# Corleone-Huang/DynamicVectorQuantization

Measured on AMD Instinct MI355X. Metric: images encoded/sec (VQ hot path: gate + routing + VQ assign), 256x256 inputs, K=1024, higher is better.
Workload: dtype f32; 1 GPU; BASELINE configs[2]: dqvae-entropy-dual-r05, B=256 per GPU, 32x32x256 latents, K=1024, entropy gate + dual routing + VectorQuantize2 assign as one op (quant_conv not in the path); global_batch=256, assign_mode=filter, spinup_steps=100, streams=3, repeats=1, full=False, parallelism=single GPU: no exchange runs, world=1, distinct_devices=1

## Files before the change

dynamicvectorquantization_amd/csrc/dvq_pass1.h:

```cpp
#pragma once
#include "dvq_filter.h"
#include <type_traits>

#define DVQ_LOAD_Z(p) __builtin_nontemporal_load(p)
#define DVQ_STORE_ZQ(p, v) __builtin_nontemporal_store((v), (p))
#define DVQ_BUF_LOAD(rsrc, voff, soff, AUX) __builtin_bit_cast(float, __builtin_amdgcn_raw_buffer_load_b32((rsrc), (voff), (soff), (AUX)))
#define DVQ_BUF_STORE(v, rsrc, voff, soff) __builtin_amdgcn_raw_buffer_store_b32(__builtin_bit_cast(unsigned, (float)(v)), (rsrc), (voff), (soff), 2)
#define DVQ_BUF_LOAD16(XT, rsrc, voff, soff, AUX) dvq_widen_bits<XT>(__builtin_amdgcn_raw_buffer_load_b16((rsrc), (voff), (soff), (AUX)))
#define DVQ_BUF_STORE16(XT, v, rsrc, voff, soff) __builtin_amdgcn_raw_buffer_store_b16(dvq_narrow_bits<XT>(v), (rsrc), (voff), (soff), 2)
#define DVQ_LOAD_SEL(p) (*(p))

#ifdef DVQ_TUNING
#ifdef __HIP_DEVICE_COMPILE__
#define DVQ_TUNING_PTR __device__
#else
#define DVQ_TUNING_PTR static __device__
#endif
DVQ_TUNING_PTR float *g_dvq_tokdbg __asm__("g_dvq_tokdbg") = nullptr;
DVQ_TUNING_PTR unsigned long long *g_dvq_stamps __asm__("g_dvq_stamps") = nullptr;
#define DVQ_STAMP(i) do { if (SPLIT && g_dvq_stamps != nullptr && threadIdx.x == 0) g_dvq_stamps[(size_t)blockIdx.x * 8 + (i)] = wall_clock64(); } while (0)
static inline int dvq_tuning_set_unit(void *stamps, void *tokdbg)
{
    int rc = (int)hipMemcpyToSymbol(HIP_SYMBOL(g_dvq_stamps), &stamps, sizeof(void *));
    if (rc) return rc;
    return (int)hipMemcpyToSymbol(HIP_SYMBOL(g_dvq_tokdbg), &tokdbg, sizeof(void *));
}
#else
#define DVQ_STAMP(i) do { } while (0)
#endif

#define DVQ_SEED_TABLE_TILES 32
constexpr size_t dvq_pass1_lds_bytes(int D) { return 4 * (size_t)(D / 16) * 1024 + 4 * 4 * 64 * sizeof(float) + 4 * 2048; }

template <int D, int SEL, bool CONV, bool FOLD, bool NT, bool RES, bool FLAT = false, bool SPLIT = false, int XT = 0>
__device__ __forceinline__ void pass1_body(
    const float *__restrict__ z, const char *__restrict__ img, const DvqF16Meta *__restrict__ meta,
    const float *__restrict__ E, const float *__restrict__ mask,
    int HW, int K, long N, float *__restrict__ zq, long long *__restrict__ codes,
    double *__restrict__ partials, int *__restrict__ counters, int *__restrict__ exact_list,
    char *__restrict__ records, int rec_cap, const DvqRouted &rv, const DvqConv &cv,
    f32x4 *__restrict__ split = nullptr, int ksplit = 1)
{
    static_assert(!SPLIT || SEL != 2, "the split form: dense or per-lane select; plain, with the conv prologue, or on the folded codebook");
    static_assert(!(SPLIT && FLAT && SEL != 0), "row-major latents are a dense op");
    static_assert(!CONV || (D == 256 && SEL != 2), "the conv prologue exists for D = 256, dense or per-lane select");
    static_assert(!(CONV && FOLD), "the conv is either computed (CONV) or folded into the code image (FOLD)");
    static_assert(!FLAT || (SEL == 0 && !CONV), "the row-major form is a dense op");
    static_assert(XT == 0 || (SEL == 0 && !CONV && !FOLD && !FLAT && !SPLIT), "16-bit latents: the dense lane-per-token form only");
    constexpr int ZB = XT ? 2 : 4;
    constexpr int NW = 4;
    constexpr int S16 = D / 16;
    constexpr int S32 = S16 / 2;
    constexpr int IMG_BYTES = S16 * 1024;
    constexpr int TILE_STRIDE = IMG_BYTES + 256;
    constexpr int CPW = (S16 + NW - 1) / NW;
    static_assert(CPW * NW == S16 && CPW <= 4, "a wave's chunks of a code tile are contiguous and within the instruction offset");
    constexpr int NBUF = 4;
    constexpr int SEED_TILES = NBUF * NW * 64 / 32;
    static_assert(SEED_TILES == DVQ_SEED_TABLE_TILES, "the launcher's limit is the table's size");
    constexpr int PER_TILE = RES ? CPW : CPW + 1;
    constexpr int FLAT_RSH = D * 2 + 16;
    constexpr int FLAT_TRW = 32 * FLAT_RSH;
    constexpr int FLAT_LPT = D * 2 / 16;
    constexpr int FLAT_TPI = 64 / FLAT_LPT;
    constexpr int FLAT_IPH = 32 / FLAT_TPI;
    static_assert(NBUF * IMG_BYTES + NBUF * NW * 64 * 4 + NW * 2048 == dvq_pass1_lds_bytes(D), "the launch's LDS is this carve");
    static_assert(!FLAT || NW * FLAT_TRW <= dvq_pass1_lds_bytes(D), "the images fit the kernel's LDS");
    extern __shared__ __attribute__((aligned(16))) char lds[];
    float *enraw = (float *)(lds + NBUF * IMG_BYTES);
    DVQ_STAMP(0);

    const int tid = threadIdx.x, lane = tid & 63;
    const int wave = __builtin_amdgcn_readfirstlane(tid >> 6);
    const int c = lane & 31, h = lane >> 5;
    const int ks = SPLIT ? (int)(blockIdx.x % (unsigned)ksplit) : 0;
    const int t_lo = SPLIT ? (int)((long)dvq_num_tiles(K) * ks / ksplit) : 0;
    const int T = SPLIT ? (int)((long)dvq_num_tiles(K) * (ks + 1) / ksplit) - t_lo : dvq_num_tiles(K);
    if constexpr (SPLIT) img += (size_t)t_lo * TILE_STRIDE;
    const float sB = meta->scale_b;
    char *scr = lds + NBUF * IMG_BYTES + NBUF * NW * 64 * 4 + wave * 2048;

    auto issue_piece = [&](int t, int q) {
        const int tt = (t < T) ? t : T - 1;
        const char *src = img + (size_t)tt * TILE_STRIDE;
        if (RES || q < CPW) {
            const char *s0 = src + wave * (CPW * 1024) + lane * 16;
            char *d0 = lds + (t & (NBUF - 1)) * IMG_BYTES + wave * (CPW * 1024);
            switch (q) {
            case 0: glds16_off<0>(s0, d0); break;
            case 1: glds16_off<1024>(s0, d0); break;
            case 2: glds16_off<2048>(s0, d0); break;
            default: glds16_off<3072>(s0, d0); break;
            }
        } else {
            glds4(src + IMG_BYTES + lane * 4, enraw + ((t & (NBUF - 1)) * NW + wave) * 64);
        }
    };
    auto issue = [&](int t) {
#pragma unroll
        for (int q = 0; q < PER_TILE; ++q) issue_piece(t, q);
    };
    auto issue_seeds = [&]() {
        if constexpr (RES) {
#pragma unroll
            for (int k = 0; k < SEED_TILES / 2 / NW; ++k) {
                const int pair = wave * (SEED_TILES / 2 / NW) + k;
                const int t0 = (2 * pair < T) ? 2 * pair : T - 1;
                const unsigned voff = (unsigned)c * 4u + ((t0 + 1 < T) ? (unsigned)h * (unsigned)TILE_STRIDE : 0u);
                glds4(img + (size_t)t0 * TILE_STRIDE + IMG_BYTES + voff, enraw + pair * 64);
            }
        }
    };
    const int tile_id = SPLIT ? (int)(blockIdx.x / (unsigned)ksplit) : xcd_swizzle(blockIdx.x, gridDim.x);
    const int pre = (SEL == 2) ? ((rv.G == 2) ? 2 : 1) : 3;

    const int n_raw = (tile_id * NW + wave) * 32 + c;
    const int n = (n_raw < N) ? n_raw : -1;
    auto token_base = [&](int HW, int h) -> size_t {
        const long nn = (n >= 0) ? n : N - 1;
        if constexpr (FLAT) return (size_t)nn * D + 8 * h;
        const long bimg = nn / HW;
        const int hw = (int)(nn - bimg * HW);
        return ((size_t)bimg * D + 8 * h) * HW + hw;
    };
    auto wave_base = [&](const float *p0, int hw, int hh) -> __amdgpu_buffer_rsrc_t {
        const size_t tb = token_base(hw, hh);
        const size_t tb0 = ((size_t)(unsigned)__builtin_amdgcn_readfirstlane((int)(tb >> 32)) << 32) |
                           (size_t)(unsigned)__builtin_amdgcn_readfirstlane((int)(tb & 0xFFFFFFFFu));
        if constexpr (XT != 0) return __builtin_amdgcn_make_buffer_rsrc((void *)((const char *)p0 + tb0 * ZB), 0, -1, 0x00020000);
        else return __builtin_amdgcn_make_buffer_rsrc((void *)(p0 + tb0), 0, -1, 0x00020000);
    };
    auto lane_off = [&](int hw, int hh) -> unsigned {
        const size_t tb = token_base(hw, hh);
        const size_t tb0 = ((size_t)(unsigned)__builtin_amdgcn_readfirstlane((int)(tb >> 32)) << 32) |
                           (size_t)(unsigned)__builtin_amdgcn_readfirstlane((int)(tb & 0xFFFFFFFFu));
        return (unsigned)(tb - tb0) * (XT ? 2u : 4u);
    };
    float zf[S16][8];
    float sel_mask = 1.0f;
    int sel_g = 0;
    unsigned stg_a = 0, stg_b = 0;
    auto conv_prologue = [&](const float *zp, size_t st) __attribute__((always_inline)) {
        constexpr int QIMG = S16 * 1024;
        constexpr int QTILE = 2 * QIMG + 256;
        float *bias_l = enraw;
        float xr[3][8];
        const float *xp = zp;
        auto issue_w = [&](int k, int q) __attribute__((always_inline)) {
            const int i = 4 * wave + q;
            glds16(cv.wimg + (size_t)(i >> 1) * QTILE + (i & 1) * QIMG + k * 1024 + lane * 16,
                   lds + (k & 3) * IMG_BYTES + i * 1024);
        };
        auto issue_x = [&](int k, int j) __attribute__((always_inline)) {
            asm volatile("global_load_dword %0, %1, off nt" : "=v"(xr[k % 3][j]) : "v"(xp) : "memory");
            xp += (j == 7) ? 9 * st : st;
        };
        auto issue_group = [&](int k) __attribute__((always_inline)) {
#pragma unroll
            for (int q = 0; q < 4; ++q) issue_w(k, q);
#pragma unroll
            for (int j = 0; j < 8; ++j) issue_x(k, j);
        };
        glds4(cv.bias + wave * 64 + lane, bias_l + wave * 64);
        issue_group(0);
        issue_group(1);
        issue_group(2);
        f32x16 acc[8];
#pragma unroll
        for (int t8 = 0; t8 < 8; ++t8)
#pragma unroll
            for (int r = 0; r < 16; ++r) acc[t8][r] = 0.0f;
        int ea = 100;
        float sa = ldexpf(1.0f, 100);
        f16x8 xh, xl;
        auto take_group = [&](int g) __attribute__((always_inline)) {
            if (g <= S16 - 3) asm volatile("s_waitcnt vmcnt(24)" ::: "memory");
            else if (g == S16 - 2) asm volatile("s_waitcnt vmcnt(12)" ::: "memory");
            else asm volatile("s_waitcnt vmcnt(0)" ::: "memory");
            float xv[8];
#pragma unroll
            for (int j = 0; j < 8; ++j) { asm volatile("" : "+v"(xr[g % 3][j])); xv[j] = xr[g % 3][j]; }
            float m = 0.0f;
#pragma unroll
            for (int j = 0; j < 8; ++j) m = vmax_abs(m, xv[j]);
            m = fmaxf(m, __shfl_xor(m, 32));
            const bool grow = (m > 0.0f) && (m < __builtin_inff()) && (m * sa >= 32768.0f);
            if (__builtin_amdgcn_ballot_w64(grow) != 0ull) {
                int e;
                (void)frexpf(grow ? m : 1.0f, &e);
                int en = 14 - e;
                en = en > 100 ? 100 : (en < -100 ? -100 : en);
                en = grow ? en : ea;
                if (g > 0) {
                    const float f = ldexpf(1.0f, en - ea);
#pragma unroll
                    for (int t8 = 0; t8 < 8; ++t8)
#pragma unroll
                        for (int r = 0; r < 16; ++r) acc[t8][r] *= f;
                }
                ea = en;
                sa = ldexpf(1.0f, ea);
            }
            u32x4 ph, pl;
#pragma unroll
            for (int j2 = 0; j2 < 4; ++j2) {
                const float v0 = xv[2 * j2] * sa, v1 = xv[2 * j2 + 1] * sa;
                const f32x2 vv = {v0, v1};
                const f16x2 hh = __builtin_convertvector(vv, f16x2);
                const f32x2 rr = {v0 - (float)hh[0], v1 - (float)hh[1]};
                const f16x2 ll = __builtin_convertvector(rr, f16x2);
                ph[j2] = __builtin_bit_cast(unsigned, hh);
                pl[j2] = __builtin_bit_cast(unsigned, ll);
            }
            xh = __builtin_bit_cast(f16x8, ph);
            xl = __builtin_bit_cast(f16x8, pl);
        };
        take_group(0);
#pragma unroll
        for (int s = 0; s < S16; ++s) {
            __builtin_amdgcn_s_barrier();
            asm volatile("" ::: "memory");
            const f16x8 bh = xh, bl = xl;
            const unsigned wa = (unsigned)(size_t)(const __attribute__((address_space(3))) char *)(lds + (s & 3) * IMG_BYTES) + lane * 16;
            f16x8 wf[3];
#define CV_OFF(Q) ((((Q) & 1) ? ((Q) - 1) : ((Q) + 1)) * 1024)
#define CV_RD(Q) asm volatile("ds_read_b128 %0, %1 offset:%c2" : "=v"(wf[(Q) % 3]) : "v"(wa), "i"(CV_OFF(Q)))
#define CV_WAIT(N, Q) asm volatile("s_waitcnt lgkmcnt(" #N ")" : "+v"(wf[(Q) % 3]) :: "memory")
            CV_RD(0); CV_RD(1); CV_RD(2);
            __builtin_amdgcn_sched_barrier(0);
#define CV_TILE(T8, W0, W1)                                                                                              \
            CV_WAIT(W0, 2 * (T8));                                                                                        \
            __builtin_amdgcn_sched_barrier(0);                                                                            \
            acc[T8] = __builtin_amdgcn_mfma_f32_32x32x16_f16(wf[(2 * (T8)) % 3], bh, acc[T8], 0, 0, 0);    \
            __builtin_amdgcn_sched_barrier(0);                                                                            \
            if (2 * (T8) + 3 < 16) { CV_RD(2 * (T8) + 3 < 16 ? 2 * (T8) + 3 : 0); }                                       \
            CV_WAIT(W1, 2 * (T8) + 1);                                                                                    \
            __builtin_amdgcn_sched_barrier(0);                                                                            \
            acc[T8] = __builtin_amdgcn_mfma_f32_32x32x16_f16(wf[(2 * (T8) + 1) % 3], bl, acc[T8], 0, 0, 0);               \
            acc[T8] = __builtin_amdgcn_mfma_f32_32x32x16_f16(wf[(2 * (T8) + 1) % 3], bh, acc[T8], 0, 0, 0);               \
            __builtin_amdgcn_sched_barrier(0);                                                                            \
            if (2 * (T8) + 4 < 16) { CV_RD(2 * (T8) + 4 < 16 ? 2 * (T8) + 4 : 0); }
#define CV_W(Q) if (s + 3 < S16) { issue_w(s + 3, Q); __builtin_amdgcn_sched_barrier(0); }
#define CV_X(J) if (s + 3 < S16) { issue_x(s + 3, J); issue_x(s + 3, (J) + 1); __builtin_amdgcn_sched_barrier(0); }
            CV_TILE(0, 2, 2) CV_W(0) CV_TILE(1, 2, 2) CV_W(1) CV_TILE(2, 2, 2) CV_W(2) CV_TILE(3, 2, 2) CV_W(3)
            CV_TILE(4, 2, 2) CV_X(0) CV_TILE(5, 2, 2) CV_X(2) CV_TILE(6, 2, 2) CV_X(4) CV_TILE(7, 1, 0) CV_X(6)
#undef CV_W
#undef CV_X
#undef CV_TILE
#undef CV_WAIT
#undef CV_RD
#undef CV_OFF
            __builtin_amdgcn_sched_barrier(0);
            if (s + 1 < S16) take_group(s + 1);
        }
        const float unscale = ldexpf(cv.meta->inv_scale_w, -ea);
#pragma unroll
        for (int s = 0; s < S16; ++s) {
            const f32x4 b0 = *(const f32x4 *)(bias_l + 16 * s + 8 * h), b1v = *(const f32x4 *)(bias_l + 16 * s + 8 * h + 4);
#pragma unroll
            for (int j = 0; j < 8; ++j)
                zf[s][j] = __builtin_fmaf(acc[s >> 1][8 * (s & 1) + j], unscale, (j < 4) ? b0[j & 3] : b1v[j & 3]);
            __builtin_amdgcn_sched_barrier(0);
        }
        if (cv.h_all && n >= 0) {
            float *hp = cv.h_buf + token_base(HW, h);
#pragma unroll
            for (int s = 0; s < S16; ++s)
#pragma unroll
                for (int j = 0; j < 8; ++j) hp[(size_t)(16 * s + j) * HW] = zf[s][j];
        }
        __builtin_amdgcn_s_barrier();
        asm volatile("" ::: "memory");
        issue_seeds();
        for (int t = 0; t < 3; ++t) issue(t);
        __builtin_amdgcn_sched_barrier(0);
    };
    if (SEL != 0) {
        const int nn = (n >= 0) ? n : (int)(N - 1);
        const int b = nn / HW, pos = nn - b * HW;
        const int y = pos / rv.Wout, x = pos - y * rv.Wout;
        const int SC = rv.sub[rv.G - 1];
        const size_t cell = (size_t)b * rv.hc * rv.wc + (y / SC) * rv.wc + x / SC;
        const DvqGateRaw graw = dvq_gate_fetch(rv.gate, rv.gate_mode, rv.G, cell);
        auto by_products = [&](int g) {
            const int rep_g = rv.rep[g];
            sel_mask = 1.0f / (float)(rep_g * rep_g);
            if (n >= 0 && h == 0 && rv.cmask_out != nullptr) {
                rv.cmask_out[n] = sel_mask;
                if (y % SC == 0 && x % SC == 0) {
                    rv.indices_out[cell] = g;
                    if (rv.gate_mode == 2 && rv.gate_out != nullptr) {
                        const float e = graw.f[0];
                        longlong2 gg; gg.x = (e <= rv.thr) ? 1 : 0; gg.y = (e > rv.thr) ? 1 : 0;
                        *(longlong2 *)(rv.gate_out + 2 * cell) = gg;
                    }
                }
            }
            if (!(y % rep_g == 0 && x % rep_g == 0)) sel_mask = -sel_mask;
        };
        if (SEL == 1) {
            const int g = dvq_gate_reduce(graw, rv.gate_mode, rv.G, rv.thr);
            by_products(g);
            int stride_l;
            const float *zp = dvq_dense_source(rv, b, y, x, g, stride_l) + (size_t)8 * h * stride_l;
            const size_t st = (size_t)stride_l;
            if constexpr (CONV) {
                conv_prologue(zp, st);
            } else {
            issue_seeds();
            for (int t = 0; t < pre; ++t) issue(t);
            __builtin_amdgcn_s_setprio(2);
#pragma unroll
            for (int s = 0; s < S16; ++s)
#pragma unroll
                for (int j = 0; j < 8; ++j) zf[s][j] = DVQ_LOAD_SEL(zp + (size_t)(16 * s + j) * st);
            __builtin_amdgcn_s_setprio(0);
            }
        } else {
            issue_seeds();
            for (int t = 0; t < pre; ++t) issue(t);
            const int bw = __builtin_amdgcn_readfirstlane(b);
            const int y0 = __builtin_amdgcn_readfirstlane(y) - wave;
            char *img_a = lds + pre * IMG_BYTES;
            char *img_b = lds + 3 * IMG_BYTES;
            {
                const int ga = rv.G - 2;
                const int plane = rv.hc * rv.sub[ga] * 16;
                const float *src = rv.src[ga] + (size_t)bw * D * plane + (size_t)(y0 >> 1) * 16 + (lane & 7) * 4;
                for (int i = wave; i < D / 8; i += NW)
                    glds16(src + (size_t)(i * 8 + (lane >> 3)) * plane, img_a + i * 1024);
            }
            if (rv.G == 3) {
                const int plane = rv.hc * 8;
                const float *src = rv.src[0] + (size_t)bw * D * plane + (size_t)(y0 >> 2) * 8 + (lane & 1) * 4;
                for (int i = wave; i < D / 32; i += NW)
                    glds16(src + (size_t)(i * 32 + (lane >> 1)) * plane, img_b + i * 1024);
            }
            stg_a = (unsigned)(size_t)(const __attribute__((address_space(3))) char *)img_a +
                    (unsigned)((8 * h) * 128 + (((wave >> 1) * 16 + (c >> 1)) << 2));
            stg_b = (unsigned)(size_t)(const __attribute__((address_space(3))) char *)img_b +
                    (unsigned)((8 * h) * 32 + ((c >> 2) << 2));
            const __amdgpu_buffer_rsrc_t zr = __builtin_amdgcn_make_buffer_rsrc((void *)(rv.src[rv.G - 1] + (size_t)bw * D * HW), 0,
                                                                                -1, 0x00020000);
            const unsigned zo = (unsigned)(8 * h * HW + pos) * 4u;
            __builtin_amdgcn_s_setprio(2);
#pragma unroll
            for (int s = 0; s < S16; ++s)
#pragma unroll
                for (int j = 0; j < 8; ++j) zf[s][j] = DVQ_BUF_LOAD(zr, zo, (16 * s + j) * HW * 4, NT ? 2 : 0);
            __builtin_amdgcn_s_setprio(0);
            asm volatile("s_waitcnt vmcnt(0)" ::: "memory");
            __builtin_amdgcn_s_barrier();
            asm volatile("" ::: "memory");
            sel_g = dvq_gate_reduce(graw, rv.gate_mode, rv.G, rv.thr);
            by_products(sel_g);
        }
    } else if constexpr (CONV) {
        conv_prologue(z + token_base(HW, h), (size_t)HW);
    } else if constexpr (FLAT) {
        char *tr = lds + wave * FLAT_TRW;
        const long n0 = ((long)tile_id * NW + wave) * 32;
        f32x4 tmp[2][FLAT_IPH];
#pragma unroll
        for (int h2 = 0; h2 < 2; ++h2)
#pragma unroll
            for (int i = 0; i < FLAT_IPH; ++i) {
                long tk = n0 + i * FLAT_TPI + lane / FLAT_LPT;
                tk = tk < N ? tk : N - 1;
                const f32x4 *src = (const f32x4 *)(z + (size_t)tk * D + h2 * (D / 2)) + (lane % FLAT_LPT);
                tmp[h2][i] = NT ? __builtin_nontemporal_load(src) : *src;
            }
#pragma unroll
        for (int h2 = 0; h2 < 2; ++h2) {
#pragma unroll
            for (int i = 0; i < FLAT_IPH; ++i)
                *(f32x4 *)(tr + (i * FLAT_TPI + lane / FLAT_LPT) * FLAT_RSH + (lane % FLAT_LPT) * 16) = tmp[h2][i];
#pragma unroll
            for (int sp = 0; sp < S16 / 2; ++sp) {
                const int s = h2 * (S16 / 2) + sp;
                const f32x4 lo = *(const f32x4 *)(tr + c * FLAT_RSH + (16 * sp + 8 * h) * 4);
                const f32x4 hi = *(const f32x4 *)(tr + c * FLAT_RSH + (16 * sp + 8 * h + 4) * 4);
#pragma unroll
                for (int j = 0; j < 4; ++j) { zf[s][j] = lo[j]; zf[s][4 + j] = hi[j]; }
            }
        }
        __syncthreads();
        issue_seeds();
        for (int t = 0; t < pre; ++t) issue(t);
    } else {
        issue_seeds();
        for (int t = 0; t < pre; ++t) issue(t);
        const __amdgpu_buffer_rsrc_t zr = wave_base(z, HW, h);
        const unsigned zo = lane_off(HW, h);
        __builtin_amdgcn_s_setprio(2);
#pragma unroll
        for (int s = 0; s < S16; ++s)
#pragma unroll
            for (int j = 0; j < 8; ++j) {
                if constexpr (XT != 0) zf[s][j] = DVQ_BUF_LOAD16(XT, zr, zo, (16 * s + j) * HW * 2, NT ? 2 : 0);
                else zf[s][j] = DVQ_BUF_LOAD(zr, zo, (16 * s + j) * HW * 4, NT ? 2 : 0);
            }
        __builtin_amdgcn_s_setprio(0);
    }
    f16x8 zb[2][S32];
    float xn, thr2W;
    unsigned copymask = 0u;
    unsigned perm_off[2] = {0u, 0u};
    if constexpr (SEL == 2) {
        copymask = (unsigned)__builtin_amdgcn_ballot_w64(sel_mask < 0.0f && h == 0);
        const int below = __builtin_popcount(copymask & ((1u << c) - 1u));
        const int p = (sel_mask < 0.0f) ? 32 - __builtin_popcount(copymask) + below : c - below;
        unsigned char *tab = (unsigned char *)scr;
        if (h == 0) tab[p] = (unsigned char)c;
#pragma unroll
        for (int t2 = 0; t2 < 2; ++t2) {
            const unsigned col = tab[16 * t2 + (lane & 15)];
            perm_off[t2] = (unsigned)(lane >> 5) * 1024u + (col + 32u * ((unsigned)(lane >> 4) & 1u)) * 16u;
        }
    }
    {
        float pa[2][8];
        float amax = 0.0f, zeta2 = 0.0f;
        f16x8 zprev = {};
#pragma unroll
        for (int s = 0; s < S16; ++s) {
            if (SEL == 2) {
                if (sel_g == rv.G - 2) {
#pragma unroll
                    for (int j = 0; j < 8; ++j)
                        asm volatile("ds_read_b32 %0, %1 offset:%c2" : "+v"(zf[s][j]) : "v"(stg_a), "i"((16 * s + j) * 128));
                    asm volatile("s_waitcnt lgkmcnt(0)" ::: "memory");
                }
                if (rv.G == 3 && sel_g == 0) {
#pragma unroll
                    for (int j = 0; j < 8; ++j)
                        asm volatile("ds_read_b32 %0, %1 offset:%c2" : "+v"(zf[s][j]) : "v"(stg_b), "i"((16 * s + j) * 32));
                    asm volatile("s_waitcnt lgkmcnt(0)" ::: "memory");
                }
#pragma unroll
                for (int j = 0; j < 8; ++j) asm volatile("" : "+v"(zf[s][j]));
            }
            u32x4 packed;
#pragma unroll
            for (int j2 = 0; j2 < 4; ++j2) {
                const float v0 = zf[s][2 * j2], v1 = zf[s][2 * j2 + 1];
                const float q0 = sq_rn(v0), q1 = sq_rn(v1);
                pa[s & 1][2 * j2] = (s < 2) ? q0 : __fadd_rn(pa[s & 1][2 * j2], q0);
                pa[s & 1][2 * j2 + 1] = (s < 2) ? q1 : __fadd_rn(pa[s & 1][2 * j2 + 1], q1);
                amax = vmax_abs(amax, v0);
                amax = vmax_abs(amax, v1);
                f32x2 vv = {v0, v1};
                f16x2 hh = __builtin_convertvector(vv, f16x2);
                packed[j2] = __builtin_bit_cast(unsigned, hh);
                const float r0 = v0 - (float)hh[0], r1 = v1 - (float)hh[1];
                zeta2 = __builtin_fmaf(r0, r0, zeta2);
                zeta2 = __builtin_fmaf(r1, r1, zeta2);
            }
            if constexpr (SEL == 2) {
                asm volatile("" : "+v"(packed), "+v"(zeta2));
                if (sel_mask < 0.0f) packed = u32x4{0u, 0u, 0u, 0u};
            }
            const f16x8 zcur = __builtin_bit_cast(f16x8, packed);
            if (s & 1) {
                const int sp = s >> 1;
                *(f16x8 *)(scr + lane * 16) = zprev;
                *(f16x8 *)(scr + 1024 + lane * 16) = zcur;
#pragma unroll
                for (int t2 = 0; t2 < 2; ++t2) {
                    if constexpr (SEL == 2) {
                        zb[t2][sp] = *(const f16x8 *)(scr + perm_off[t2]);
                    } else {
                    const int srcl = 16 * t2 + (lane & 15) + 32 * ((lane >> 4) & 1);
                    zb[t2][sp] = *(const f16x8 *)(scr + (lane >> 5) * 1024 + srcl * 16);
                    }
                }
            }
            zprev = zcur;
            if constexpr (CONV) __builtin_amdgcn_sched_barrier(0);
        }
        float t8[8];
#pragma unroll
        for (int l = 0; l < 8; ++l) {
            float o0 = __shfl_xor(pa[0][l], 32), o1 = __shfl_xor(pa[1][l], 32);
            float a0 = h == 0 ? pa[0][l] : o0;
            float a1 = h == 0 ? o0 : pa[0][l];
            float a2 = h == 0 ? pa[1][l] : o1;
            float a3 = h == 0 ? o1 : pa[1][l];
            t8[l] = __fadd_rn(__fadd_rn(__fadd_rn(a0, a1), a2), a3);
        }
        xn = t8[0];
#pragma unroll
        for (int l = 1; l < 8; ++l) xn = __fadd_rn(xn, t8[l]);
        amax = fmaxf(amax, __shfl_xor(amax, 32));
        zeta2 += __shfl_xor(zeta2, 32);
        thr2W = FOLD ? dvq_fold_threshold(xn, amax, zeta2, sB, (const DvqFoldMeta *)meta)
                     : dvq_filter_threshold(xn, amax, zeta2, sB, meta);
    }
    if (SEL == 2) {
        __builtin_amdgcn_s_barrier();
        asm volatile("" ::: "memory");
    }
    for (int t = pre; t < 3; ++t) issue(t);
    DVQ_STAMP(1);

    float best, second;
    int code;
    {
        const int q16 = lane >> 4;
        float b1[2] = {-__builtin_inff(), -__builtin_inff()}, b2[2] = {-__builtin_inff(), -__builtin_inff()};
        int bt[2] = {0, 0};
        if constexpr (SEL == 2) {
            if (__builtin_popcount(copymask) >= 16) {
#define DVQ_NG 1
#include "pass1_loop.h"
#undef DVQ_NG
            } else {
#define DVQ_NG 2
#include "pass1_loop.h"
#undef DVQ_NG
            }
        } else {
#define DVQ_NG 2
#include "pass1_loop.h"
#undef DVQ_NG
        }
        asm volatile("s_waitcnt vmcnt(0)" ::: "memory");
        float rb[2], rs[2];
        int rc[2];
#pragma unroll
        for (int t2 = 0; t2 < 2; ++t2) {
            float mb = b1[t2], ms = b2[t2];
            int mt = bt[t2], mq = q16;
#pragma unroll
            for (int off = 16; off <= 32; off <<= 1) {
                const float o1 = __shfl_xor(mb, off), o2 = __shfl_xor(ms, off);
                const int ot = __shfl_xor(mt, off), oq = __shfl_xor(mq, off);
                const bool other_wins = (o1 > mb) || (o1 == mb && ((lane ^ off) < lane));
                ms = fmaxf(other_wins ? mb : o1, fmaxf(ms, o2));
                mb = other_wins ? o1 : mb;
                mt = other_wins ? ot : mt;
                mq = other_wins ? oq : mq;
            }
            const int r = (int)(__float_as_uint(mb) & 15u);
            rb[t2] = mb;
            rs[t2] = ms;
            rc[t2] = (mt + t_lo) * 32 + 16 * (r >> 2) + 4 * mq + (r & 3);
        }
        if constexpr (SEL == 2) {
            unsigned cm = copymask;
            asm volatile("" : "+s"(cm));
            const int c_p = (int)__builtin_amdgcn_mbcnt_hi(~0u, __builtin_amdgcn_mbcnt_lo(~0u, 0u)) & 31;
            const int below = __builtin_popcount(cm & ((1u << c_p) - 1u));
            const int pc = ((cm >> c_p) & 1u) ? 32 - __builtin_popcount(cm) + below : c_p - below;
            const int srcl = pc & 15;
            const float x0 = __shfl(rb[0], srcl), x1 = __shfl(rb[1], srcl);
            const float y0 = __shfl(rs[0], srcl), y1 = __shfl(rs[1], srcl);
            const int c0 = __shfl(rc[0], srcl), c1 = __shfl(rc[1], srcl);
            best = (pc >> 4) ? x1 : x0;
            second = (pc >> 4) ? y1 : y0;
            code = (pc >> 4) ? c1 : c0;
        } else {
        const int srcl = c & 15;
        const float x0 = __shfl(rb[0], srcl), x1 = __shfl(rb[1], srcl);
        const float y0 = __shfl(rs[0], srcl), y1 = __shfl(rs[1], srcl);
        const int c0 = __shfl(rc[0], srcl), c1 = __shfl(rc[1], srcl);
        best = (c >> 4) ? x1 : x0;
        second = (c >> 4) ? y1 : y0;
        code = (c >> 4) ? c1 : c0;
        }
    }
    DVQ_STAMP(2);
    if constexpr (SEL == 2) {
        const int lane_e = (int)__builtin_amdgcn_mbcnt_hi(~0u, __builtin_amdgcn_mbcnt_lo(~0u, 0u));
        const int c_e = lane_e & 31;
        float am = __builtin_fabsf(sel_mask);
        asm volatile("" : "+v"(am));
        const int rm1 = (am == 1.0f) ? 0 : ((am == 0.25f) ? 1 : 3);
        char *hand = lds + NBUF * IMG_BYTES + NBUF * NW * 64 * 4;
        if (lane_e < 32) {
            const f32x4 mine = {best, second, __int_as_float(code), 0.0f};
            *(f32x4 *)(hand + wave * 2048 + c_e * 16) = mine;
        }
        __syncthreads();
        const f32x4 own = *(const f32x4 *)(hand + (wave - (wave & rm1)) * 2048 + (c_e - (c_e & rm1)) * 16);
        best = own[0];
        second = own[1];
        code = __float_as_int(own[2]);
    }
    if constexpr (SPLIT) {
        typedef __attribute__((address_space(1))) unsigned long long gu64;
        __shared__ int s_last;
        gu64 *mine = (gu64 *)(split + ((size_t)tile_id * ksplit) * 128 + wave * 32 + c);
        if (h == 0) {
            gu64 *e = mine + (size_t)ks * 128 * 2;
            __hip_atomic_store(e, ((unsigned long long)__float_as_uint(second) << 32) | __float_as_uint(best), __ATOMIC_RELAXED, __HIP_MEMORY_SCOPE_AGENT);
            __hip_atomic_store(e + 1, (unsigned long long)(unsigned)code, __ATOMIC_RELAXED, __HIP_MEMORY_SCOPE_AGENT);
        }
        asm volatile("s_waitcnt vmcnt(0)" ::: "memory");
        __syncthreads();
        DVQ_STAMP(3);
        if (tid == 0) {
            const int old = __hip_atomic_fetch_add(&counters[DVQ_SPLIT_TICKET0 + tile_id], 1, __ATOMIC_RELAXED, __HIP_MEMORY_SCOPE_AGENT);
            s_last = (old == ksplit - 1);
            if (old == ksplit - 1)
                __hip_atomic_store(&counters[DVQ_SPLIT_TICKET0 + tile_id], 0, __ATOMIC_RELAXED, __HIP_MEMORY_SCOPE_AGENT);
        }
        __syncthreads();
        DVQ_STAMP(4);
        if (!s_last) return;
        float mb = -__builtin_inff(), ms = -__builtin_inff();
        int mc = 0;
        unsigned long long e0[DVQ_SPLIT_MAX_SLICES], e1[DVQ_SPLIT_MAX_SLICES];
#pragma unroll
        for (int k = 0; k < DVQ_SPLIT_MAX_SLICES; ++k) {
            const int kk = k < ksplit ? k : ksplit - 1;
            e0[k] = __hip_atomic_load(mine + (size_t)kk * 128 * 2, __ATOMIC_RELAXED, __HIP_MEMORY_SCOPE_AGENT);
            e1[k] = __hip_atomic_load(mine + (size_t)kk * 128 * 2 + 1, __ATOMIC_RELAXED, __HIP_MEMORY_SCOPE_AGENT);
        }
#pragma unroll
        for (int k = 0; k < DVQ_SPLIT_MAX_SLICES; ++k) {
            const float eb = __uint_as_float((unsigned)e0[k]), es = __uint_as_float((unsigned)(e0[k] >> 32));
            const bool other_wins = k < ksplit && eb > mb;
            ms = (k < ksplit) ? fmaxf(other_wins ? mb : eb, fmaxf(ms, es)) : ms;
            mc = other_wins ? (int)(unsigned)e1[k] : mc;
            mb = other_wins ? eb : mb;
        }
        best = mb; second = ms; code = mc;
        DVQ_STAMP(5);
    }
    const float thr = best - thr2W;
    const bool final_ok = (best - second) > thr2W;
    const bool valid = n >= 0;
    bool hopeless = !(code < K) || !(thr == thr);
#ifdef DVQ_TUNING
    if (g_dvq_tokdbg != nullptr && valid && h == 0) {
        f32x4 dbg = {best, second, thr2W, (float)code};
        *(f32x4 *)(g_dvq_tokdbg + 4 * (size_t)n) = dbg;
    }
#endif
    const bool undecided = valid && !hopeless && !final_ok;
    const int sel_rep = (SEL == 0 || sel_mask < 0.0f) ? (SEL == 0 ? 1 : 0) : (sel_mask == 1.0f ? 1 : (sel_mask == 0.25f ? 2 : 4));
    const bool queued = undecided && sel_rep > 0;
    const unsigned long long umask = __ballot(queued && h == 0);
    const int shard = (SPLIT ? tile_id * NW + wave : (int)blockIdx.x) & (DVQ_QSHARDS - 1);
    int slot_raw = 0;
    if (umask != 0ull && lane == 0) slot_raw = atomicAdd(&counters[DVQ_QCOUNT0 + shard], (int)__popcll(umask));
    if (valid && hopeless && h == 0) {
        int pos = atomicAdd(&counters[DVQ_C_EXACT], 1);
        exact_list[pos] = n;
    }
    float lsum = 0.0f;
    float m_tok = 1.0f;
    if (valid && !hopeless) {
        if (h == 0) codes[n] = (long long)code;
        m_tok = (SEL != 0) ? __builtin_fabsf(sel_mask) : ((mask != nullptr) ? mask[n] : 1.0f);
        if (zq != nullptr || partials != nullptr) {
            int h_e = h;
            if constexpr (FOLD || (FLAT && SPLIT) || SEL == 2) h_e =(int)(__builtin_amdgcn_mbcnt_hi(~0u, __builtin_amdgcn_mbcnt_lo(~0u, 0u)) >> 5);
            const float *ep = E + (size_t)code * D + 8 * h_e;
            constexpr int SB = SPLIT ? ((S16 < 8) ? S16 : 8) : ((S16 < 2) ? S16 : 2);
            auto finish = [&](auto store_tag) {
                constexpr bool STORE = decltype(store_tag)::value;
                int hw_e = HW;
                asm volatile("" : "+s"(hw_e));
                const __amdgpu_buffer_rsrc_t qr = wave_base(STORE ? zq : (float *)E, hw_e, h_e);
                const unsigned qo = lane_off(hw_e, h_e);
                int hw4 = HW * (XT ? 2 : 4);
                asm volatile("" : "+s"(hw4));
#pragma unroll
                for (int s0 = 0; s0 < S16; s0 += SB) {
                    f32x4 eg[SB][2];
#pragma unroll
                    for (int q = 0; q < SB; ++q) {
                        eg[q][0] = *(const f32x4 *)(ep + 16 * (s0 + q));
                        eg[q][1] = *(const f32x4 *)(ep + 16 * (s0 + q) + 4);
                    }
#pragma unroll
                    for (int q = 0; q < SB; ++q) {
                        const int s = s0 + q;
#pragma unroll
                        for (int j = 0; j < 8; ++j) {
                            float e = eg[q][j >> 2][j & 3];
                            if constexpr (FOLD) {
                                if (STORE) DVQ_BUF_STORE(e, qr, qo, (16 * s + j) * hw4);
                            } else {
                            float diff = __fsub_rn(e, zf[s][j]);
                            if constexpr (XT != 0) {
                                if (STORE) DVQ_BUF_STORE16(XT, __fadd_rn(zf[s][j], diff), qr, qo, (16 * s + j) * hw4);
                            } else
                            if (STORE) DVQ_BUF_STORE(__fadd_rn(zf[s][j], diff), qr, qo, (16 * s + j) * hw4);
                            lsum = __builtin_fmaf(diff, diff, lsum);
                            }
                        }
                    }
                }
            };
            if constexpr (!FLAT) {
                if (zq != nullptr) finish(std::true_type{});
                else finish(std::false_type{});
                lsum *= m_tok;
            }
        }
    }
    if constexpr (FLAT) {
        char *flat_tr = lds + wave * FLAT_TRW;
        const bool store = zq != nullptr;
        if (store) __syncthreads();
        const bool mine = valid && !hopeless && (store || partials != nullptr);
        const unsigned long long okmask = __ballot(valid && !hopeless && h == 0);
        const long n0 = ((long)tile_id * NW + wave) * 32;
        const float *ep = E + (size_t)(mine ? code : 0) * D + 8 * h;
#pragma unroll
        for (int h2 = 0; h2 < 2; ++h2) {
            if (mine) {
                constexpr int SB = (S16 / 2 < 2) ? S16 / 2 : 2;
#pragma unroll
                for (int sp0 = 0; sp0 < S16 / 2; sp0 += SB) {
                    f32x4 eg[SB][2];
#pragma unroll
                    for (int q = 0; q < SB; ++q) {
                        eg[q][0] = *(const f32x4 *)(ep + 16 * (h2 * (S16 / 2) + sp0 + q));
                        eg[q][1] = *(const f32x4 *)(ep + 16 * (h2 * (S16 / 2) + sp0 + q) + 4);
                    }
#pragma unroll
                    for (int q = 0; q < SB; ++q) {
                        const int sp = sp0 + q, s = h2 * (S16 / 2) + sp;
                        f32x4 o[2];
#pragma unroll
                        for (int j = 0; j < 8; ++j) {
                            const float e = eg[q][j >> 2][j & 3];
                            if constexpr (FOLD) {
                                o[j >> 2][j & 3] = e;
                            } else {
                                const float diff = __fsub_rn(e, zf[s][j]);
                                o[j >> 2][j & 3] = __fadd_rn(zf[s][j], diff);
                                lsum = __builtin_fmaf(diff, diff, lsum);
                            }
                        }
                        if (store) {
                            *(f32x4 *)(flat_tr + c * FLAT_RSH + (16 * sp + 8 * h) * 4) = o[0];
                            *(f32x4 *)(flat_tr + c * FLAT_RSH + (16 * sp + 8 * h + 4) * 4) = o[1];
                        }
                    }
                }
            }
            if (store) {
#pragma unroll
                for (int i = 0; i < FLAT_IPH; ++i) {
                    const int tk = i * FLAT_TPI + lane / FLAT_LPT;
                    const f32x4 v = *(const f32x4 *)(flat_tr + tk * FLAT_RSH + (lane % FLAT_LPT) * 16);
                    if ((okmask >> tk) & 1ull)
                        __builtin_nontemporal_store(v, (f32x4 *)(zq + (size_t)(n0 + tk) * D + h2 * (D / 2)) + (lane % FLAT_LPT));
                }
            }
        }
        lsum *= m_tok;
    }
    DVQ_STAMP(6);
    if (umask != 0ull) {
        const int base = __shfl(slot_raw, 0);
        int slot = base + (int)__popcll(umask & ((1ull << c) - 1ull));
        slot = queued ? slot : -1;
        if (queued && slot >= rec_cap) {
            if (h == 0) {
                const int rr = sel_rep > 0 ? sel_rep : 1;
                for (int ry = 0; ry < rr; ++ry)
                    for (int rx = 0; rx < rr; ++rx) {
                        int pos = atomicAdd(&counters[DVQ_C_EXACT], 1);
                        exact_list[pos] = n + ry * rv.Wout + rx;
                    }
            }
            lsum = -(float)(sel_rep * sel_rep - 1) * lsum;
            slot = -1;
        }
        if (slot >= 0) {
            char *rec = records + ((size_t)shard * rec_cap + slot) * rec_bytes(D);
#pragma unroll
            for (int s = 0; s < S16; ++s) {
                f32x4 lo = {zf[s][0], zf[s][1], zf[s][2], zf[s][3]};
                f32x4 hi = {zf[s][4], zf[s][5], zf[s][6], zf[s][7]};
                *(f32x4 *)(rec + (16 * s + 8 * h) * 4) = lo;
                *(f32x4 *)(rec + (16 * s + 8 * h + 4) * 4) = hi;
            }
            if (h == 0) {
                RecMeta rm;
                rm.n = n; rm.xn = xn; rm.thr = thr; rm.m = m_tok; rm.prov = code;
                rm.best = ~0ull; rm.rep = sel_rep > 0 ? sel_rep : 1;
                *(RecMeta *)(rec + (size_t)D * 4) = rm;
            }
        }
    }
    if (partials != nullptr) {
        double dsum = (double)lsum;
#pragma unroll
        for (int off = 32; off > 0; off >>= 1) dsum += __shfl_xor(dsum, off);
        __syncthreads();
        double *red = (double *)lds;
        if (lane == 0) red[wave] = dsum;
        __syncthreads();
        if (tid == 0) partials[SPLIT ? tile_id : (int)blockIdx.x] = (red[0] + red[1]) + (red[2] + red[3]);
    }
    DVQ_STAMP(7);
}

template <int D, int SEL, bool CONV, bool FOLD, bool RES>
__global__ __launch_bounds__(256, 2) void vq_assign_filter_kernel(
    const float *__restrict__ z, const char *__restrict__ img, const DvqF16Meta *__restrict__ meta,
    const float *__restrict__ E, const float *__restrict__ mask,
    int HW, int K, long N, float *__restrict__ zq, long long *__restrict__ codes,
    double *__restrict__ partials, int *__restrict__ counters, int *__restrict__ exact_list,
    char *__restrict__ records, int rec_cap, const DvqRouted rv, const DvqConv cv)
{
    pass1_body<D, SEL, CONV, FOLD, true, RES>(z, img, meta, E, mask, HW, K, N, zq, codes, partials, counters, exact_list, records, rec_cap, rv, cv);
}

template <int D, bool FOLD, bool RES>
__global__ __launch_bounds__(256, 2) void vq_assign_filter_flat_kernel(
    const float *__restrict__ z, const char *__restrict__ img, const DvqF16Meta *__restrict__ meta,
    const float *__restrict__ E, const float *__restrict__ mask,
    int HW, int K, long N, float *__restrict__ zq, long long *__restrict__ codes,
    double *__restrict__ partials, int *__restrict__ counters, int *__restrict__ exact_list,
    char *__restrict__ records, int rec_cap, const DvqRouted rv, const DvqConv cv)
{
    pass1_body<D, 0, false, FOLD, true, RES, true>(z, img, meta, E, mask, HW, K, N, zq, codes, partials, counters, exact_list, records, rec_cap, rv, cv);
}

template <int D, int SEL, bool CONV, bool FOLD, bool FLAT, bool RES>
__global__ __launch_bounds__(256, 2) void vq_assign_filter_split_kernel(
    const float *__restrict__ z, const char *__restrict__ img, const DvqF16Meta *__restrict__ meta,
    const float *__restrict__ E, const float *__restrict__ mask,
    int HW, int K, long N, float *__restrict__ zq, long long *__restrict__ codes,
    double *__restrict__ partials, int *__restrict__ counters, int *__restrict__ exact_list,
    char *__restrict__ records, int rec_cap, const DvqRouted rv, const DvqConv cv, f32x4 *__restrict__ split, int ksplit)
{
    pass1_body<D, SEL, CONV, FOLD, CONV, RES, FLAT, true>(z, img, meta, E, mask, HW, K, N, zq, codes, partials, counters, exact_list, records,
                                                     rec_cap, rv, cv, split, ksplit);
}

template <int D, int SEL, bool FOLD, bool RES>
__global__ __launch_bounds__(256, 2) void vq_assign_filter_cached_kernel(
    const float *__restrict__ z, const char *__restrict__ img, const DvqF16Meta *__restrict__ meta,
    const float *__restrict__ E, const float *__restrict__ mask,
    int HW, int K, long N, float *__restrict__ zq, long long *__restrict__ codes,
    double *__restrict__ partials, int *__restrict__ counters, int *__restrict__ exact_list,
    char *__restrict__ records, int rec_cap, const DvqRouted rv, const DvqConv cv)
{
    pass1_body<D, SEL, false, FOLD, false, RES>(z, img, meta, E, mask, HW, K, N, zq, codes, partials, counters, exact_list, records, rec_cap, rv, cv);
}

template <int D, bool RES, int XT>
__global__ __launch_bounds__(256, 2) void vq_assign_filter_x16_kernel(
    const void *__restrict__ z, const char *__restrict__ img, const DvqF16Meta *__restrict__ meta,
    const float *__restrict__ E, const float *__restrict__ mask,
    int HW, int K, long N, void *__restrict__ zq, long long *__restrict__ codes,
    double *__restrict__ partials, int *__restrict__ counters, int *__restrict__ exact_list,
    char *__restrict__ records, int rec_cap)
{
    static_assert(XT == 1 || XT == 2, "f16 or bf16");
    pass1_body<D, 0, false, false, true, RES, false, false, XT>((const float *)z, img, meta, E, mask, HW, K, N, (float *)zq, codes, partials,
                                                                counters, exact_list, records, rec_cap, DvqRouted{}, DvqConv{});
}

struct FilterWs {
    int *counters, *chunk_sync, *exact_list;
    char *records;
    int cap;
    f32x4 *split;
};

enum class P1Form { plain, cached, flat, split, wide, x16 };
struct P1Plan {
    P1Form form;
    int sel;
    bool conv, fold, flat;
    int ks;
    int xt;
};

constexpr bool p1_keeps_seed_piece(int D, P1Form form, bool fold, bool flat)
{
    return D == 256 && ((form == P1Form::flat && fold) || (form == P1Form::split && flat));
}

struct P1Args {
    const float *z;
    const char *img16;
    const DvqF16Meta *meta;
    const float *E, *mask;
    int HW, K;
    long N;
// ... 103 lines not shown
```

dynamicvectorquantization_amd/csrc/pass1_loop.h:

```cpp
        f32x4 acc16[2][2];
        auto top2 = [&](int tt) {
#pragma unroll
            for (int t2 = 0; t2 < DVQ_NG; ++t2) {
                const float om = b1[t2];
#pragma unroll
                for (int r = 0; r < 8; r += 2) {
                    const float v0 = acc16[r >> 2][t2][r & 3], v1 = acc16[(r + 1) >> 2][t2][(r + 1) & 3];
                    float g0 = __uint_as_float((__float_as_uint(v0) & 0xFFFFFFF0u) | (unsigned)r);
                    float g1 = __uint_as_float((__float_as_uint(v1) & 0xFFFFFFF0u) | (unsigned)(r + 1));
                    float md = __builtin_amdgcn_fmed3f(b1[t2], g0, g1);
                    b1[t2] = vmax3_raw(b1[t2], g0, g1);
                    b2[t2] = vmax_raw(b2[t2], md);
                }
                bt[t2] = (b1[t2] != om) ? tt : bt[t2];
            }
        };
    for (int t = 0; t < T; ++t) {
            asm volatile("s_waitcnt vmcnt(%0)" ::"n"(PER_TILE) : "memory");
            __builtin_amdgcn_s_barrier();
            asm volatile("" ::: "memory");
            if (S16 != 16) issue(t + 3);
            const unsigned tile_a = (unsigned)(size_t)(const __attribute__((address_space(3))) char *)(
                                        lds + (t & (NBUF - 1)) * IMG_BYTES + lane * 16);
            f16x8 a0, a1, a2, a3;
#define DVQ_RD(dst, S) asm volatile("ds_read_b128 %0, %1 offset:%c2" : "=v"(dst) : "v"(tile_a), "i"((S) * 1024))
            DVQ_RD(a0, 0); DVQ_RD(a1, 1); DVQ_RD(a2, 2); DVQ_RD(a3, 3);
            __builtin_amdgcn_sched_barrier(0);
            if (t > 0) top2(t - 1);
            __builtin_amdgcn_sched_barrier(0);
            {
                const unsigned seed_a = (unsigned)(size_t)(const __attribute__((address_space(3))) char *)(
                                            RES ? enraw + t * 32 + 4 * q16 : enraw + ((t & (NBUF - 1)) * NW + wave) * 64 + 4 * q16);
                f32x4 e0, e1;
                asm volatile("ds_read_b128 %0, %1" : "=v"(e0) : "v"(seed_a));
                asm volatile("ds_read_b128 %0, %1 offset:64" : "=v"(e1) : "v"(seed_a));
                asm volatile("s_waitcnt lgkmcnt(0)" : "+v"(e0), "+v"(e1), "+v"(a0), "+v"(a1), "+v"(a2), "+v"(a3) :: "memory");
                acc16[0][0] = e0; if (DVQ_NG == 2) acc16[0][1] = e0;
                acc16[1][0] = e1; if (DVQ_NG == 2) acc16[1][1] = e1;
            }
            __builtin_amdgcn_sched_barrier(0);
#define DVQ_PIECE(Q) if constexpr ((Q) < PER_TILE) { issue_piece(t + 3, Q); }
#define DVQ_MM(src, F, WAIT, NEXT)                                                                             \
            asm volatile("s_waitcnt lgkmcnt(" #WAIT ")" ::: "memory");                                            \
            __builtin_amdgcn_sched_barrier(0);                                                                    \
            acc16[(F) / S32][0] = __builtin_amdgcn_mfma_f32_16x16x32_f16(src, zb[0][(F) % S32], acc16[(F) / S32][0], 0, 0, 0); \
            if (DVQ_NG == 2)                                                                                      \
            acc16[(F) / S32][1] = __builtin_amdgcn_mfma_f32_16x16x32_f16(src, zb[1][(F) % S32], acc16[(F) / S32][1], 0, 0, 0); \
            __builtin_amdgcn_sched_barrier(0);                                                                    \
            if ((F) + 4 < S16) { DVQ_RD(src, ((F) + 4 < S16 ? (F) + 4 : 0)); }                                  \
            NEXT
            __builtin_amdgcn_s_setprio(1);
            if (S16 == 16) {
                DVQ_MM(a0, 0, 0, ) DVQ_MM(a1, 1, 1, DVQ_PIECE(0)) DVQ_MM(a2, 2, 2, ) DVQ_MM(a3, 3, 3, )
                DVQ_MM(a0, 4, 3, DVQ_PIECE(1)) DVQ_MM(a1, 5, 3, ) DVQ_MM(a2, 6, 3, ) DVQ_MM(a3, 7, 3, DVQ_PIECE(2))
                DVQ_MM(a0, 8, 3, ) DVQ_MM(a1, 9, 3, ) DVQ_MM(a2, 10, 3, DVQ_PIECE(3)) DVQ_MM(a3, 11, 3, )
                DVQ_MM(a0, 12, 3, ) DVQ_MM(a1, 13, 2, DVQ_PIECE(4)) DVQ_MM(a2, 14, 1, ) DVQ_MM(a3, 15, 0, )
            } else if (S16 == 8) {
                DVQ_MM(a0, 0, 0, ) DVQ_MM(a1, 1, 1, ) DVQ_MM(a2, 2, 2, ) DVQ_MM(a3, 3, 3, )
                DVQ_MM(a0, 4, 3, ) DVQ_MM(a1, 5, 2, ) DVQ_MM(a2, 6, 1, ) DVQ_MM(a3, 7, 0, )
            } else {
                DVQ_MM(a0, 0, 0, ) DVQ_MM(a1, 1, 0, ) DVQ_MM(a2, 2, 0, ) DVQ_MM(a3, 3, 0, )
            }
#undef DVQ_MM
#undef DVQ_RD
#undef DVQ_PIECE
            __builtin_amdgcn_s_setprio(0);
        }
        top2(T - 1);
```

Measured before the change: 1.343 million images/s.

## Compact real tokens across the workgroup to skip MFMA work for copied tokens

For the SEL==2, D==256 path, each wave publishes its copy-token mask to shared memory. Real (non-copied) tokens are then compacted across all four waves through an LDS exchange buffer, so each wave runs the codebook distance loop only on its share of the compacted tokens (0, 1 or 2 MFMA groups). Results are scattered back through LDS to the owning lanes. This removes wasted MFMA work when many tokens are duplicates, at the cost of extra workgroup barriers and LDS traffic in the transpose and hand-back phases.

```diff
diff --git a/dynamicvectorquantization_amd/csrc/dvq_pass1.h b/dynamicvectorquantization_amd/csrc/dvq_pass1.h
--- a/dynamicvectorquantization_amd/csrc/dvq_pass1.h
+++ b/dynamicvectorquantization_amd/csrc/dvq_pass1.h
@@ -112,7 +112,18 @@
         }
     };
     const int tile_id = SPLIT ? (int)(blockIdx.x / (unsigned)ksplit) : xcd_swizzle(blockIdx.x, gridDim.x);
+    constexpr bool WGC = (SEL == 2 && D == 256);
     const int pre = (SEL == 2) ? ((rv.G == 2) ? 2 : 1) : 3;
+    char *const xbuf_a = lds + NBUF * IMG_BYTES + NBUF * NW * 64 * 4;
+    char *xbuf_b = nullptr;
+    if constexpr (WGC) xbuf_b = lds + pre * IMG_BYTES;
+    static_assert(!WGC || (64 * 128 == 8192 && S32 >= 4), "channels 0 .. 63 of the [D][32 floats] image are the second buffer");
+    unsigned wgm0 = 0u, wgm1 = 0u, wgm2 = 0u, wgm3 = 0u;
+    unsigned *wg_masks = nullptr;
+    if constexpr (WGC) {
+        __shared__ unsigned s_wg_masks[4];
+        wg_masks = s_wg_masks;
+    }
 
     const int n_raw = (tile_id * NW + wave) * 32 + c;
     const int n = (n_raw < N) ? n_raw : -1;
@@ -349,11 +360,24 @@
 #pragma unroll
                 for (int j = 0; j < 8; ++j) zf[s][j] = DVQ_BUF_LOAD(zr, zo, (16 * s + j) * HW * 4, NT ? 2 : 0);
             __builtin_amdgcn_s_setprio(0);
+            if constexpr (WGC) {
+                sel_g = dvq_gate_reduce(graw, rv.gate_mode, rv.G, rv.thr);
+                const int rep_g = rv.rep[sel_g];
+                const unsigned cm = (unsigned)__builtin_amdgcn_ballot_w64(!(y % rep_g == 0 && x % rep_g == 0) && h == 0);
+                if (lane == 0) wg_masks[wave] = cm;
+                asm volatile("s_waitcnt vmcnt(0) lgkmcnt(0)" ::: "memory");
+            } else
             asm volatile("s_waitcnt vmcnt(0)" ::: "memory");
             __builtin_amdgcn_s_barrier();
             asm volatile("" ::: "memory");
-            sel_g = dvq_gate_reduce(graw, rv.gate_mode, rv.G, rv.thr);
+            if constexpr (!WGC) sel_g = dvq_gate_reduce(graw, rv.gate_mode, rv.G, rv.thr);
             by_products(sel_g);
+            if constexpr (WGC) {
+                wgm0 = (unsigned)__builtin_amdgcn_readfirstlane((int)wg_masks[0]);
+                wgm1 = (unsigned)__builtin_amdgcn_readfirstlane((int)wg_masks[1]);
+                wgm2 = (unsigned)__builtin_amdgcn_readfirstlane((int)wg_masks[2]);
+                wgm3 = (unsigned)__builtin_amdgcn_readfirstlane((int)wg_masks[3]);
+            }
         }
     } else if constexpr (CONV) {
         conv_prologue(z + token_base(HW, h), (size_t)HW);
@@ -406,6 +430,32 @@
     float xn, thr2W;
     unsigned copymask = 0u;
     unsigned perm_off[2] = {0u, 0u};
+    int ng = 2;
+    if constexpr (WGC) {
+        const int nr0 = 32 - __builtin_popcount(wgm0), nr1 = 32 - __builtin_popcount(wgm1), nr2 = 32 - __builtin_popcount(wgm2);
+        const int pf1 = nr0, pf2 = pf1 + nr1, pf3 = pf2 + nr2, nreal_wg = pf3 + 32 - __builtin_popcount(wgm3);
+        const int left = nreal_wg - 32 * wave + 15;
+        ng = __builtin_amdgcn_readfirstlane(left < 16 ? 0 : (left < 32 ? 1 : 2));
+        const int wz = wgm0 ? 0 : (wgm1 ? 1 : (wgm2 ? 2 : 3));
+        const unsigned mz = wgm0 ? wgm0 : (wgm1 ? wgm1 : (wgm2 ? wgm2 : wgm3));
+        const int cz = mz ? __builtin_ctz(mz) : 0;
+#pragma unroll
+        for (int t2 = 0; t2 < 2; ++t2) {
+            const int P = 32 * wave + 16 * t2 + (lane & 15);
+            const int ws = (P >= pf3) ? 3 : ((P >= pf2) ? 2 : ((P >= pf1) ? 1 : 0));
+            int k = P - ((P >= pf3) ? pf3 : ((P >= pf2) ? pf2 : ((P >= pf1) ? pf1 : 0)));
+            const unsigned real = ~((ws == 3) ? wgm3 : ((ws == 2) ? wgm2 : ((ws == 1) ? wgm1 : wgm0)));
+            int col = 0;
+#pragma unroll
+            for (int sh = 16; sh >= 1; sh >>= 1) {
+                const int cnt = __builtin_popcount((real >> col) & ((1u << sh) - 1u));
+                if (k >= cnt) { k -= cnt; col += sh; }
+            }
+            const bool past = P >= nreal_wg;
+            const unsigned wsrc = past ? (unsigned)wz : (unsigned)ws, csrc = past ? (unsigned)cz : (unsigned)col;
+            perm_off[t2] = wsrc * 2048u + (unsigned)(lane >> 5) * 1024u + (csrc + 32u * ((unsigned)(lane >> 4) & 1u)) * 16u;
+        }
+    } else
     if constexpr (SEL == 2) {
         copymask = (unsigned)__builtin_amdgcn_ballot_w64(sel_mask < 0.0f && h == 0);
         const int below = __builtin_popcount(copymask & ((1u << c) - 1u));
@@ -463,6 +513,21 @@
             const f16x8 zcur = __builtin_bit_cast(f16x8, packed);
             if (s & 1) {
                 const int sp = s >> 1;
+                if constexpr (WGC) {
+                    char *xb = (sp >= 2 && !(sp & 1)) ? xbuf_b : xbuf_a;
+                    if (sp == 1) {
+                        asm volatile("s_waitcnt lgkmcnt(0)" ::: "memory");
+                        __builtin_amdgcn_s_barrier();
+                        asm volatile("" ::: "memory");
+                    }
+                    *(f16x8 *)(xb + wave * 2048 + lane * 16) = zprev;
+                    *(f16x8 *)(xb + wave * 2048 + 1024 + lane * 16) = zcur;
+                    asm volatile("s_waitcnt lgkmcnt(0)" ::: "memory");
+                    __builtin_amdgcn_s_barrier();
+                    asm volatile("" ::: "memory");
+#pragma unroll
+                    for (int t2 = 0; t2 < 2; ++t2) zb[t2][sp] = *(const f16x8 *)(xb + perm_off[t2]);
+                } else {
                 *(f16x8 *)(scr + lane * 16) = zprev;
                 *(f16x8 *)(scr + 1024 + lane * 16) = zcur;
 #pragma unroll
@@ -474,6 +539,7 @@
                     zb[t2][sp] = *(const f16x8 *)(scr + (lane >> 5) * 1024 + srcl * 16);
                     }
                 }
+                }
             }
             zprev = zcur;
             if constexpr (CONV) __builtin_amdgcn_sched_barrier(0);
@@ -497,6 +563,7 @@
                      : dvq_filter_threshold(xn, amax, zeta2, sB, meta);
     }
     if (SEL == 2) {
+        if constexpr (WGC) asm volatile("s_waitcnt lgkmcnt(0)" ::: "memory");
         __builtin_amdgcn_s_barrier();
         asm volatile("" ::: "memory");
     }
@@ -509,6 +576,21 @@
         const int q16 = lane >> 4;
         float b1[2] = {-__builtin_inff(), -__builtin_inff()}, b2[2] = {-__builtin_inff(), -__builtin_inff()};
         int bt[2] = {0, 0};
+        if constexpr (WGC) {
+            if (ng == 0) {
+#define DVQ_NG 0
+#include "pass1_loop.h"
+#undef DVQ_NG
+            } else if (ng == 1) {
+#define DVQ_NG 1
+#include "pass1_loop.h"
+#undef DVQ_NG
+            } else {
+#define DVQ_NG 2
+#include "pass1_loop.h"
+#undef DVQ_NG
+            }
+        } else
         if constexpr (SEL == 2) {
             if (__builtin_popcount(copymask) >= 16) {
 #define DVQ_NG 1
@@ -546,6 +628,17 @@
             rs[t2] = ms;
             rc[t2] = (mt + t_lo) * 32 + 16 * (r >> 2) + 4 * mq + (r & 3);
         }
+        if constexpr (WGC) {
+            const int lane_t = (int)__builtin_amdgcn_mbcnt_hi(~0u, __builtin_amdgcn_mbcnt_lo(~0u, 0u));
+            if (lane_t < 16) {
+#pragma unroll
+                for (int t2 = 0; t2 < 2; ++t2) {
+                    const f32x4 mine = {rb[t2], rs[t2], __int_as_float(rc[t2]), 0.0f};
+                    *(f32x4 *)(xbuf_a + (32 * wave + 16 * t2 + lane_t) * 16) = mine;
+                }
+            }
+            best = 0.0f; second = 0.0f; code = 0;
+        } else
         if constexpr (SEL == 2) {
             unsigned cm = copymask;
             asm volatile("" : "+s"(cm));
@@ -577,6 +670,20 @@
         asm volatile("" : "+v"(am));
         const int rm1 = (am == 1.0f) ? 0 : ((am == 0.25f) ? 1 : 3);
         char *hand = lds + NBUF * IMG_BYTES + NBUF * NW * 64 * 4;
+        if constexpr (WGC) {
+            unsigned m0 = wgm0, m1 = wgm1, m2 = wgm2, m3 = wgm3;
+            asm volatile("" : "+s"(m0), "+s"(m1), "+s"(m2), "+s"(m3));
+            const int wave_o = wave - (wave & rm1), c_o = c_e - (c_e & rm1);
+            const int q1 = 32 - __builtin_popcount(m0), q2 = q1 + 32 - __builtin_popcount(m1), q3 = q2 + 32 - __builtin_popcount(m2);
+            const unsigned m_o = (wave_o == 0) ? m0 : ((wave_o == 1) ? m1 : ((wave_o == 2) ? m2 : m3));
+            const int pf_o = (wave_o == 0) ? 0 : ((wave_o == 1) ? q1 : ((wave_o == 2) ? q2 : q3));
+            const int p_o = pf_o + __builtin_popcount(~m_o & ((1u << c_o) - 1u));
+            __syncthreads();
+            const f32x4 own = *(const f32x4 *)(hand + p_o * 16);
+            best = own[0];
+            second = own[1];
+            code = __float_as_int(own[2]);
+        } else {
         if (lane_e < 32) {
             const f32x4 mine = {best, second, __int_as_float(code), 0.0f};
             *(f32x4 *)(hand + wave * 2048 + c_e * 16) = mine;
@@ -586,6 +693,7 @@
         best = own[0];
         second = own[1];
         code = __float_as_int(own[2]);
+        }
     }
     if constexpr (SPLIT) {
         typedef __attribute__((address_space(1))) unsigned long long gu64;
diff --git a/dynamicvectorquantization_amd/csrc/pass1_loop.h b/dynamicvectorquantization_amd/csrc/pass1_loop.h
--- a/dynamicvectorquantization_amd/csrc/pass1_loop.h
+++ b/dynamicvectorquantization_amd/csrc/pass1_loop.h
@@ -1,3 +1,4 @@
+#if DVQ_NG != 0
         f32x4 acc16[2][2];
         auto top2 = [&](int tt) {
 #pragma unroll
@@ -15,11 +16,16 @@
                 bt[t2] = (b1[t2] != om) ? tt : bt[t2];
             }
         };
+#endif
     for (int t = 0; t < T; ++t) {
             asm volatile("s_waitcnt vmcnt(%0)" ::"n"(PER_TILE) : "memory");
             __builtin_amdgcn_s_barrier();
             asm volatile("" ::: "memory");
             if (S16 != 16) issue(t + 3);
+#if DVQ_NG == 0
+            if (S16 == 16) issue(t + 3);
+        }
+#else
             const unsigned tile_a = (unsigned)(size_t)(const __attribute__((address_space(3))) char *)(
                                         lds + (t & (NBUF - 1)) * IMG_BYTES + lane * 16);
             f16x8 a0, a1, a2, a3;
@@ -67,3 +73,4 @@
             __builtin_amdgcn_s_setprio(0);
         }
         top2(T - 1);
+#endif
```

Result: faster. 1.378 million images/s (median of 6 runs) (+2.7%).
